# dernasherbrezon/sdr-server

Hardware: AMD Instinct MI355X
Metric: input IQ Msamples/s processed (all clients), 2.016 Msps->48 kHz xlating FIR (higher is better)
Workload: dtype f32; 1 GPU; 1024 clients x 48 kHz off one 2.016 Msps cu8 stream, D=42, 505 taps, 262144-byte blocks (BASELINE configs[3]; N=1: the >=1000-client single-GPU target); clients_total=1024, clients_per_gpu=1024, blocks_per_call=8, mode=optimized, parallelism=single GPU, rccl_ranks=1, feed=xlating_multi (C host)

## Files before the change

### sdr-server_amd/csrc/xl_dev_inline.h

```cpp
#ifndef XL_DEV_INLINE_H_
#define XL_DEV_INLINE_H_
#include "xl_device.h"
#include "xl_q15_narrow.h"

typedef float v2f __attribute__((ext_vector_type(2)));
typedef float v4f __attribute__((ext_vector_type(4)));
typedef const float __attribute__((address_space(4))) *cfloat_p;
typedef const uint32_t __attribute__((address_space(4))) *cu32_p;

#define XL_DEV static __device__ __forceinline__
#define XL_MEM __device__ __forceinline__

XL_DEV v2f xl_sample(const void *__restrict__ p, int fmt, uint32_t i) {
  v2f r;
  if (fmt == XLF_CU8) {
    const uint32_t v = reinterpret_cast<const uint16_t *>(p)[i];
    r.x = ((float)(v & 0xFFu) - 127.5f) / 128.0f;
    r.y = ((float)(v >> 8) - 127.5f) / 128.0f;
  } else if (fmt == XLF_CS8) {
    const int32_t v = reinterpret_cast<const int16_t *>(p)[i];
    r.x = (float)((int32_t)(int8_t)(v & 0xFF)) / 128.0f;
    r.y = (float)(v >> 8) / 128.0f;
  } else if (fmt == XLF_CS16) {
    const int32_t v = reinterpret_cast<const int32_t *>(p)[i];
    r.x = (float)((int32_t)(int16_t)(v & 0xFFFF)) / 32768.0f;
    r.y = (float)(v >> 16) / 32768.0f;
  } else {
    r = reinterpret_cast<const v2f *>(p)[i];
  }
  return r;
}

XL_DEV v2f xl_sample_q15(const void *__restrict__ p, int fmt, uint32_t i) {
  v2f r;
  if (fmt == XLF_CU8) {
    const uint32_t v = reinterpret_cast<const uint16_t *>(p)[i];
    r.x = (float)(((int32_t)(v & 0xFFu) - 128) * 256);
    r.y = (float)(((int32_t)(v >> 8) - 128) * 256);
  } else if (fmt == XLF_CS8) {
    const int32_t v = reinterpret_cast<const int16_t *>(p)[i];
    r.x = (float)((int32_t)(int8_t)(v & 0xFF) * 256);
    r.y = (float)((v >> 8) * 256);
  } else {
    const int32_t v = reinterpret_cast<const int32_t *>(p)[i];
    r.x = (float)(int32_t)(int16_t)(v & 0xFFFF);
    r.y = (float)(v >> 16);
  }
  return r;
}

XL_DEV void xl_q15_rotate_store(const short2 *__restrict__ qphtab, float2 *out, uint32_t off, uint32_t qi, uint32_t m, int32_t ar,
                                int32_t ai) {
  const short2 p0 = qphtab[(off >> XL_PH_SHIFT) + (m >> XL_PH_SHIFT)];
  const int32_t ir = (int16_t)(qi & 0xFFFFu), ii = (int16_t)(qi >> 16);
  int32_t pr = p0.x, pi = p0.y;
  for (uint32_t j = m & (XL_PH_STRIDE - 1u); j > 0u; --j) {
    const int32_t tr = pr * ir - pi * ii, ti = pr * ii + pi * ir;
    pr = xl_sat16(tr >> 15);
    pi = xl_sat16(ti >> 15);
  }
  const int32_t orr = ar * pr - ai * pi, oi = ar * pi + ai * pr;
  reinterpret_cast<short2 *>(out + off)[m] = make_short2((short)xl_sat16(orr >> 15), (short)xl_sat16(oi >> 15));
}

template <int MODE>
struct XlAcc;

template <>
struct XlAcc<0> {
  v2f s;
  XL_MEM void clear() { s = (v2f){0.0f, 0.0f}; }
  XL_MEM void mac(const v2f x, const float hr, const float hi) {
    const v2f h = {hr, hi};
    v2f p1, p2;
    asm("v_pk_mul_f32 %0, %3, %4 op_sel_hi:[0,1]\n\t"
        "v_pk_mul_f32 %1, %3, %4 op_sel:[1,1] op_sel_hi:[1,0]\n\t"
        "v_pk_add_f32 %0, %0, %1 neg_lo:[0,1]\n\t"
        "v_pk_add_f32 %2, %2, %0"
        : "=&v"(p1), "=&v"(p2), "+v"(s)
        : "v"(x), "s"(h));
  }
  XL_MEM v2f value() const { return s; }
};

template <>
struct XlAcc<1> {
  v2f a, b;
  XL_MEM void clear() {
    a = (v2f){0.0f, 0.0f};
    b = (v2f){0.0f, 0.0f};
  }
  XL_MEM void mac(const v2f x, const float hr, const float hi) {
    a = __builtin_elementwise_fma((v2f){x.x, x.x}, (v2f){hr, hi}, a);
    b = __builtin_elementwise_fma((v2f){x.y, x.y}, (v2f){hi, hr}, b);
  }
  XL_MEM v2f value() const { return (v2f){a.x - b.x, a.y + b.y}; }
};

template <int MODE>
XL_DEV v2f xl_rotate(const v2f a, const v2f p) {
  v2f r;
  if (MODE == 0) {
    r.x = a.x * p.x - a.y * p.y;
    r.y = a.x * p.y + a.y * p.x;
  } else {
    r.x = __builtin_fmaf(-a.y, p.y, a.x * p.x);
    r.y = __builtin_fmaf(a.y, p.x, a.x * p.y);
  }
  return r;
}

XL_DEV void xl_nco_step(v2f &p, const v2f inc) {
  v2f t1, t2;
  asm volatile(
      "v_pk_mul_f32 %0, %2, %3 op_sel_hi:[1,0]\n\t"
      "v_pk_mul_f32 %1, %2, %3 op_sel:[0,1] op_sel_hi:[1,1]"
      : "=&v"(t1), "=&v"(t2)
      : "v"(p), "v"(inc));
  asm volatile("v_pk_add_f32 %0, %1, %2 op_sel:[0,1] op_sel_hi:[1,0] neg_lo:[0,1]" : "=v"(p) : "v"(t1), "v"(t2));
}

XL_DEV v2f xl_nco_next(const v2f p, const v2f inc) {
  v2f t1, t2, r;
  asm volatile(
      "v_pk_mul_f32 %0, %3, %4 op_sel_hi:[1,0]\n\t"
      "v_pk_mul_f32 %1, %3, %4 op_sel:[0,1] op_sel_hi:[1,1]\n\t"
      "v_pk_add_f32 %2, %0, %1 op_sel:[0,1] op_sel_hi:[1,0] neg_lo:[0,1]"
      : "=&v"(t1), "=&v"(t2), "=&v"(r)
      : "v"(p), "v"(inc));
  return r;
}

XL_DEV v2f xl_nco_next_fma(const v2f p, const v2f inc) {
  v2f t, r;
  asm volatile(
      "v_pk_mul_f32 %0, %2, %3 op_sel:[1,1] op_sel_hi:[1,0]\n\t"
      "v_pk_fma_f32 %1, %2, %3, %0 op_sel_hi:[0,1,1] neg_lo:[0,0,1]"
      : "=&v"(t), "=&v"(r)
      : "v"(p), "v"(inc));
  return r;
}
XL_DEV v2f xl_nco_next_any(const v2f p, const v2f inc, const uint32_t flags) {
  return (flags & XL_POS_FMA_STEP) ? xl_nco_next_fma(p, inc) : xl_nco_next(p, inc);
}

XL_DEV v2f xl_nco_role_step(const v2f p, const v2f inc, const uint32_t flags) {
  float a, b, c, d;
  if (flags & XL_POS_FMA_STEP) {
    asm volatile(
        "v_mul_f32 %0, %3, %5\n\t"
        "v_mul_f32 %1, %3, %4\n\t"
        "v_fma_f32 %0, %2, %4, -%0\n\t"
        "v_fma_f32 %1, %2, %5, %1"
        : "=&v"(a), "=&v"(b)
        : "v"(p.x), "v"(p.y), "v"(inc.x), "v"(inc.y));
    return (v2f){a, b};
  }
  asm volatile(
      "v_mul_f32 %0, %4, %6\n\t"
      "v_mul_f32 %1, %5, %7\n\t"
      "v_mul_f32 %2, %4, %7\n\t"
      "v_mul_f32 %3, %5, %6\n\t"
      "v_sub_f32 %0, %0, %1\n\t"
      "v_add_f32 %1, %3, %2"
// ... 87 lines not shown
```

### sdr-server_amd/csrc/xl_kernels.hip

```cpp
#include "xl_dev_inline.h"
#include "xl_chain_plan.h"

#include <hip/hip_ext.h>

#include <stdlib.h>

__global__ __launch_bounds__(64) void xl_nco_table_kernel(const XlNcoClient *__restrict__ cl, uint32_t n,
                                                          const float2 *state_in, float2 *state_out,
                                                          float2 *__restrict__ tab, const XlPos pos,
                                                          const uint32_t explicit_K, const uint32_t prio,
                                                          const uint32_t lanes) {
  if (prio == 3) __builtin_amdgcn_s_setprio(3);
  else if (prio == 2) __builtin_amdgcn_s_setprio(2);
  else if (prio == 1) __builtin_amdgcn_s_setprio(1);
  if (threadIdx.x >= lanes) return;
  const uint32_t c = blockIdx.x * lanes + threadIdx.x;
  if (c >= n) return;
  const XlNcoClient k = cl[c];
  const XlBnd bnd = xl_nco_bnd(k, pos, explicit_K);
  asm volatile("" ::: "v255", "a255");
  xl_nco_client_chain<true>(k, bnd, 0u, bnd.K, state_in, state_out, tab);
}

#define XLC_RING 64u
XL_DEV uint32_t xl_lds_off(const void *p) { return (uint32_t)(uintptr_t)(__attribute__((address_space(3))) const char *)p; }
XL_DEV void xl_lds_post(const uint32_t addr, const uint32_t v) { asm volatile("ds_write_b32 %0, %1" ::"v"(addr), "v"(v) : "memory"); }
XL_DEV void xl_lds_post64(const uint32_t addr, const v2f v) { asm volatile("ds_write_b64 %0, %1" ::"v"(addr), "v"(v) : "memory"); }
XL_DEV uint32_t xl_lds_poll(const uint32_t addr) {
  uint32_t v;
  asm volatile("ds_read_b32 %0, %1\n\ts_waitcnt lgkmcnt(0)" : "=v"(v) : "v"(addr) : "memory");
  return v;
}

XL_DEV uint32_t xl_lds_poll3_min(const uint32_t a0, const uint32_t a1, const uint32_t a2) {
  uint32_t v0, v1, v2;
  asm volatile("ds_read_b32 %0, %3\n\tds_read_b32 %1, %4\n\tds_read_b32 %2, %5\n\ts_waitcnt lgkmcnt(0)"
               : "=&v"(v0), "=&v"(v1), "=&v"(v2)
               : "v"(a0), "v"(a1), "v"(a2)
               : "memory");
  v0 = v0 < v1 ? v0 : v1;
  return v0 < v2 ? v0 : v2;
}
XL_DEV uint32_t xl_chain_lim(const uint32_t mn) { return mn >= 0x7FFFFFE0u ? 0xFFFFFFFFu : 2u * mn + XLC_RING; }
XL_DEV uint32_t xl_chain_wait_drained(const uint32_t upto, const uint32_t a0, const uint32_t a1, const uint32_t a2) {
  uint32_t lim = 0u;
  for (uint32_t spin = 0; spin < (1u << 22); ++spin) {
    lim = xl_chain_lim((uint32_t)__builtin_amdgcn_readfirstlane((int)xl_lds_poll3_min(a0, a1, a2)));
    if (upto <= lim) break;
    __builtin_amdgcn_s_sleep(1);
  }
  return lim;
}
XL_DEV uint32_t xl_chain_event(uint32_t ev) {
  const unsigned long long act = __ballot(ev != 0xFFFFFFFFu);
  if (act == 0ull) return 0xFFFFFFFFu;
  const uint32_t first = (uint32_t)__builtin_amdgcn_readlane((int)ev, (int)__ffsll((long long)act) - 1);
  if (__ballot(ev != 0xFFFFFFFFu && ev != first) == 0ull) return first;
#pragma unroll
  for (int sh = 1; sh < 64; sh <<= 1) {
    const uint32_t other = (uint32_t)__shfl_xor((int)ev, sh);
    ev = other < ev ? other : ev;
  }
  return (uint32_t)__builtin_amdgcn_readfirstlane((int)ev);
}

#define XLC_ALIGN ".p2align 6\n\t"
#define XLC_MUL "v_pk_mul_f32 %[t1], %[p], %[inc] op_sel_hi:[1,0]\n\tv_pk_mul_f32 %[t2], %[p], %[inc] op_sel:[0,1] op_sel_hi:[1,1]\n\t"
#define XLC_ADD "v_pk_add_f32 %[p], %[t1], %[t2] op_sel:[0,1] op_sel_hi:[1,0] neg_lo:[0,1]\n\t"
#define XLC_STEP XLC_MUL XLC_ADD
#define XLC_STEP2(I1, I2) XLC_MUL I1 "\n\t" XLC_ADD I2 "\n\t"
#define XLC_STEPS10 XLC_STEP XLC_STEP XLC_STEP XLC_STEP XLC_STEP XLC_STEP XLC_STEP XLC_STEP XLC_STEP XLC_STEP
#define XLC_ANY_LOOP                                                                       \
  "1:\n\t" XLC_MUL "ds_write_b64 %[addr], %[p]\n\t" XLC_ADD                               \
  XLC_STEP2("v_add_u32 %[cnt], 1, %[cnt]", "s_sub_u32 %[todo], %[todo], 1")               \
  XLC_MUL "ds_write_b32 %[paddr], %[cnt]\n\t" XLC_ADD                                     \
  XLC_MUL "v_add_u32 %[off], 0x200, %[off]\n\t" XLC_ADD                                   \
  XLC_MUL "v_and_b32 %[off], 0x7fff, %[off]\n\t" XLC_ADD                                  \
  XLC_STEP2("v_add_u32 %[addr], %[off], %[base]", "s_cmp_lg_u32 %[todo], 0")              \
  XLC_STEPS10 "s_cbranch_scc1 1b\n\t"
#define XLC_B8_LOOP                                                                        \
  "2:\n\t" XLC_E7("0", "512", "1024", "1536", "2048", "2560", "3072")                    \
  XLC_MUL "ds_write_b64 %[addr], %[p] offset:3584\n\t" XLC_ADD                           \
  XLC_STEP2("v_add_u32 %[cnt], 8, %[cnt]", "s_sub_u32 %[todo8], %[todo8], 1")            \
  XLC_MUL "ds_write_b32 %[paddr], %[cnt]\n\t" XLC_ADD                                    \
  XLC_MUL "v_add_u32 %[off], 0x1000, %[off]\n\t" XLC_ADD                                 \
  XLC_MUL "v_and_b32 %[off], 0x7fff, %[off]\n\t" XLC_ADD                                 \
  XLC_STEP2("v_add_u32 %[addr], %[off], %[base]", "s_cmp_lg_u32 %[todo8], 0")            \
  XLC_STEPS10 "s_cbranch_scc1 2b\n\t"
#define XLC_ANY_PART "s_cmp_eq_u32 %[todo], 0\n\ts_cbranch_scc1 3f\n\t" XLC_ANY_LOOP "3:\n\ts_nop 0\n\t"
#define XLC_B8_PART "s_cmp_eq_u32 %[todo8], 0\n\ts_cbranch_scc1 4f\n\t" XLC_B8_LOOP "4:\n\ts_nop 0\n\t"
#define XLC_STEP_LOOP "1:\n\t" XLC_STEP2("s_sub_u32 %[todo], %[todo], 1", "s_cmp_lg_u32 %[todo], 0") "s_cbranch_scc1 1b\n\t"
#define XLC_QENTRY(OFFS) XLC_MUL "ds_write_b64 %[addr], %[p] offset:" OFFS "\n\t" XLC_ADD XLC_STEP XLC_STEP
#define XLC_E(OFFS) XLC_QENTRY(OFFS) XLC_STEP XLC_STEP XLC_STEP XLC_STEPS10
#define XLC_E7(B0, B1, B2, B3, B4, B5, B6) XLC_E(B0) XLC_E(B1) XLC_E(B2) XLC_E(B3) XLC_E(B4) XLC_E(B5) XLC_E(B6)
#define XLC_E8(B0, B1, B2, B3, B4, B5, B6, B7) XLC_E7(B0, B1, B2, B3, B4, B5, B6) XLC_E(B7)
#define XLC_B32_LOOP                                                                                         \
  XLC_E8("0", "512", "1024", "1536", "2048", "2560", "3072", "3584")                                       \
  XLC_E8("4096", "4608", "5120", "5632", "6144", "6656", "7168", "7680")                                   \
  XLC_E8("8192", "8704", "9216", "9728", "10240", "10752", "11264", "11776")                               \
  XLC_E("12288") XLC_E("12800") XLC_E("13312") XLC_E("13824") XLC_E("14336") XLC_E("14848")               \
  XLC_QENTRY("15360")                                                                                      \
  XLC_MUL "ds_read_b32 %[mn], %[an0]\n\t" XLC_ADD                                                           \
  XLC_MUL "ds_read_b32 %[n1], %[an1]\n\t" XLC_ADD                                                           \
  XLC_MUL "ds_read_b32 %[n2], %[an2]\n\t" XLC_ADD XLC_STEPS10                                               \
  XLC_MUL "ds_write_b64 %[addr], %[p] offset:15872\n\t" XLC_ADD                                             \
  XLC_MUL "v_add_u32 %[cnt], 32, %[cnt]\n\t" XLC_ADD "s_sub_u32 %[todo], %[todo], 1\n\t"                    \
  XLC_MUL "ds_write_b32 %[paddr], %[cnt]\n\t" XLC_ADD                                                       \
  XLC_MUL "v_add_u32 %[off], 0x4000, %[off]\n\t" XLC_ADD                                                    \
  XLC_MUL "v_and_b32 %[off], 0x7fff, %[off]\n\t" XLC_ADD                                                    \
  XLC_STEP2("v_add_u32 %[addr], %[off], %[base]", "s_add_u32 %[need], %[need], 16")                         \
  XLC_STEP2("s_waitcnt lgkmcnt(0)", "v_min_u32 %[mn], %[mn], %[n1]")                                        \
  XLC_STEP2("v_min_u32 %[mn], %[mn], %[n2]", "s_nop 0")                                                     \
  XLC_STEP2("v_readfirstlane_b32 %[sm], %[mn]", "s_nop 0")                                                  \
  XLC_STEP2("s_cmp_ge_u32 %[sm], %[need]", "s_cselect_b32 %[st], %[todo], 0")                               \
  XLC_STEP XLC_STEP XLC_STEP XLC_STEP XLC_STEP XLC_STEP
static_assert(XL_PH_STRIDE == 16u && XLC_RING * 64u * 8u == 0x8000u, "the chain wave's asm blocks are written for 16 steps per entry and a 32 KB ring");

__global__ __launch_bounds__(256) void xl_nco_chain_kernel(const XlNcoClient *__restrict__ cl, uint32_t n,
                                                           const float2 *state_in, const XlChainCalls calls,
                                                           XlPos pos, unsigned long long *stats) {
  asm volatile("" ::: "v255", "a255");
  const unsigned long long t_entry = stats ? wall_clock64() : 0ull;
  __shared__ v2f ring[XLC_RING][64];
  __shared__ uint32_t s_emax;
  __shared__ uint32_t s_prod;
  __shared__ uint32_t s_next[3];
  const uint32_t w = __builtin_amdgcn_readfirstlane(threadIdx.x >> 6), lane = threadIdx.x & 63u;
  const uint32_t c = blockIdx.x * 64u + lane;
  const bool have = c < n;
  XlNcoClient k;
  k.incr = make_float2(1.0f, 0.0f);
  k.out_off = 0u, k.slot = 0u, k.D = 1u, k.rem0 = 0u;
  if (have) k = cl[c];
  v2f p = {1.0f, 0.0f};
  if (w == 0 && have) p = (v2f){state_in[k.slot].x, state_in[k.slot].y};
  unsigned long long cyc = 0ull, ticks = 0ull, wfirst = 0ull;
  uint32_t entries = 0u;
  for (uint32_t call = 0; call < calls.n; ++call, pos = xl_grid_next(pos)) {
    float2 *const tab = calls.tab[call];
    float2 *const state_out = calls.state_out[call];
    if (call) __syncthreads();
    XlBnd bnd = xl_nco_bnd(k, pos, 0xFFFFFFFFu);
    if (!have) bnd.K = 0u;
    const uint32_t K = bnd.K, E = (K + XL_PH_STRIDE - 1u) >> XL_PH_SHIFT;
    if (threadIdx.x == 0) {
      s_emax = 0u;
      s_prod = 0u;
      s_next[0] = 0u, s_next[1] = 1u, s_next[2] = 2u;
    }
    __syncthreads();
    if (w == 0 && E > 0u) atomicMax(&s_emax, E);
    __syncthreads();
    const uint32_t Emax = (uint32_t)__builtin_amdgcn_readfirstlane((int)s_emax);
    const uint32_t a_prod = xl_lds_off(&s_prod), a_ring0 = xl_lds_off(&ring[0][0]), a_ring = xl_lds_off(&ring[0][lane]);
    v2f *__restrict__ o = reinterpret_cast<v2f *>(tab) + (k.out_off >> XL_PH_SHIFT);
    if (w == 0) {
      __builtin_amdgcn_s_setprio(3);
      const v2f inc = {k.incr.x, k.incr.y};
      uint32_t nb = xl_bnd_next(bnd, 0u);
      const uint32_t a_n0 = xl_lds_off(&s_next[0]), a_n1 = xl_lds_off(&s_next[1]), a_n2 = xl_lds_off(&s_next[2]);
      const unsigned long long c0 = stats ? clock64() : 0ull, w0 = stats ? wall_clock64() : 0ull;
      unsigned long long t_region = 0ull, t_drain = 0ull, t_b32 = 0ull;
      uint32_t n_drain = 0u, n_b32 = 0u, n_event = 0u, n_runs = 0u;
      uint32_t e = 0;
      uint32_t lim = XLC_RING;
      uint32_t evs = xl_chain_event(0u < K ? (nb < K ? nb : K) : 0xFFFFFFFFu);
      while (e < Emax) {
        uint32_t e_stop = evs == 0u ? 0u : (evs - 1u) >> XL_PH_SHIFT;
        e_stop = e_stop < Emax ? e_stop : Emax;
        if (pos.pad & XL_POS_FMA_STEP) e_stop = e;
        const unsigned long long r0 = stats ? clock64() : 0ull;
        if ((e << XL_PH_SHIFT) < K) {
          const XlChainPlan8 pl = xl_chain_plan8(e, e_stop, XLC_RING, 32u, 8u);
          uint32_t ee = e;
          v2f t1, t2;
#define XLC_COVER_RUN(N1, N8, PARTS)                                                                                         \
  if ((N1) + (N8) != 0u) {                                                                                                   \
    uint32_t todo = (N1), todo8 = (N8);                                                                                      \
    const uint32_t total = todo + 8u * todo8;                                                                                \
    if (ee + total > lim) {                                                                                                  \
      const unsigned long long d0 = stats ? clock64() : 0ull;                                                                \
      lim = xl_chain_wait_drained(ee + total, a_n0, a_n1, a_n2);                                                             \
      if (stats) t_drain += clock64() - d0, ++n_drain;                                                                       \
    }                                                                                                                        \
    uint32_t off = ((ee & (XLC_RING - 1u)) << 9) + lane * (uint32_t)sizeof(v2f);     \
    uint32_t addr = a_ring0 + off, cnt = ee;                                                                                 \
    ee += total;                                                                                                             \
    asm volatile(XLC_ALIGN PARTS                                                                                             \
                 : [p] "+v"(p), [off] "+v"(off), [addr] "+v"(addr), [cnt] "+v"(cnt), [t1] "=&v"(t1), [t2] "=&v"(t2),         \
                   [todo] "+s"(todo), [todo8] "+s"(todo8)                                                                    \
                 : [inc] "v"(inc), [base] "v"(a_ring0), [paddr] "v"(a_prod)                                                  \
                 : "memory", "scc");                                                                                         \
  }
          XLC_COVER_RUN(pl.head1, pl.head8, XLC_ANY_PART XLC_B8_PART);
          for (uint32_t want = pl.blocks; want != 0u;) {
            if (ee + 32u > lim) {
              const unsigned long long d0 = stats ? clock64() : 0ull;
              lim = xl_chain_wait_drained(ee + 32u, a_n0, a_n1, a_n2);
              if (stats) t_drain += clock64() - d0, ++n_drain;
            }
            uint32_t off = ((ee & (XLC_RING - 1u)) << 9) + lane * (uint32_t)sizeof(v2f);
            uint32_t addr = a_ring0 + off, cnt = ee;
            uint32_t left = want, need = (ee >> 1) - 16u, mn, n1, n2, sm, st;
            const unsigned long long b0 = stats ? clock64() : 0ull;
            asm volatile(XLC_ALIGN "1:\n\t" XLC_B32_LOOP "s_cmp_lg_u32 %[st], 0\n\ts_cbranch_scc1 1b\n\t"
                         : [p] "+v"(p), [off] "+v"(off), [addr] "+v"(addr), [cnt] "+v"(cnt), [t1] "=&v"(t1), [t2] "=&v"(t2),
                           [mn] "=&v"(mn), [n1] "=&v"(n1), [n2] "=&v"(n2), [todo] "+s"(left), [need] "+s"(need), [sm] "=&s"(sm),
                           [st] "=&s"(st)
                         : [inc] "v"(inc), [base] "v"(a_ring0), [paddr] "v"(a_prod), [an0] "v"(a_n0), [an1] "v"(a_n1), [an2] "v"(a_n2)
                         : "memory", "scc");
            const uint32_t ran = (want - left) << 5;
            if (stats) t_b32 += clock64() - b0, n_b32 += ran, ++n_runs;
            lim = xl_chain_lim(sm);
            ee += ran;
            want = left;
          }
          XLC_COVER_RUN(pl.tail1, pl.tail8, XLC_B8_PART XLC_ANY_PART);
#undef XLC_COVER_RUN
        }
        if (e_stop > e) e = e_stop;
        if (stats) t_region += clock64() - r0, ++n_event;
        if (e < Emax) {
          if (e + 1u > lim) lim = xl_chain_wait_drained(e + 1u, a_n0, a_n1, a_n2);
          const uint32_t m0 = e << XL_PH_SHIFT;
          if (m0 < K) xl_lds_post64(a_ring + (e & (XLC_RING - 1u)) * 64u * (uint32_t)sizeof(v2f), p);
          xl_lds_post(a_prod, e + 1u);
          uint32_t m = m0;
          if (!(pos.pad & XL_POS_FMA_STEP) && evs - m0 - 1u < XL_PH_STRIDE &&
              __ballot(m0 < K && (nb != evs || m0 + XL_PH_STRIDE > K)) == 0ull && m0 < K) {
            v2f t1, t2;
            uint32_t todo = evs - m0;
            asm volatile(XLC_ALIGN XLC_STEP_LOOP
                         : [p] "+v"(p), [t1] "=&v"(t1), [t2] "=&v"(t2), [todo] "+s"(todo)
                         : [inc] "v"(inc)
                         : "scc");
            p = xl_nco_renorm(p);
            nb = xl_bnd_next(bnd, evs);
            m = evs;
            todo = m0 + XL_PH_STRIDE - evs;
            if (todo != 0u && __ballot(nb <= m0 + XL_PH_STRIDE) == 0ull) {
              asm volatile(XLC_ALIGN XLC_STEP_LOOP
                           : [p] "+v"(p), [t1] "=&v"(t1), [t2] "=&v"(t2), [todo] "+s"(todo)
                           : [inc] "v"(inc)
                           : "scc");
              m = m0 + XL_PH_STRIDE;
            }
          }
          for (; m < m0 + XL_PH_STRIDE && m < K; ++m) {
            p = xl_nco_next_any(p, inc, bnd.flags);
            if (m + 1u == nb) {
              p = xl_nco_renorm(p);
              nb = xl_bnd_next(bnd, m + 1u);
            }
          }
          ++e;
          evs = xl_chain_event((e << XL_PH_SHIFT) < K ? (nb < K ? nb : K) : 0xFFFFFFFFu);
        }
      }
      if (have) state_out[k.slot] = make_float2(p.x, p.y);
      if (stats) {
        cyc += clock64() - c0;
        const unsigned long long w1 = wall_clock64();
        ticks += w1 - w0;
        entries += Emax;
        if (call == 0u) wfirst = w0;
        if (lane == 0u && blockIdx.x < 1024u) {
          stats[8192u + 8u * blockIdx.x + 1u + 2u * call] = w0 - t_entry;
          stats[8192u + 8u * blockIdx.x + 2u + 2u * call] = w1 - t_entry;
        }
        if (lane == 0u && blockIdx.x < 128u) {
          unsigned long long *const sp = stats + 4096u + 32u * blockIdx.x + 8u * call;
          const unsigned long long k0 = clock64(), k1 = clock64(), k2 = clock64(), k3 = clock64(), k4 = clock64();
          (void)k1, (void)k2, (void)k3;
          sp[0] = k0 - c0, sp[1] = t_region, sp[2] = t_drain, sp[3] = t_b32;
          sp[4] = n_drain, sp[5] = n_b32, sp[6] = n_event | ((unsigned long long)n_runs << 32), sp[7] = (k4 - k0) / 4ull;
        }
      }
      continue;
    }
    const uint32_t j = w - 1u;
    const uint32_t a_next = xl_lds_off(&s_next[j]);
    v4f *__restrict__ o4 = reinterpret_cast<v4f *>(o);
    for (uint32_t q = j; 2u * q < Emax; q += 3u) {
      const uint32_t need = 2u * q + 2u < Emax ? 2u * q + 2u : Emax;
      for (uint32_t spin = 0; spin < (1u << 24); ++spin) {
        if (xl_lds_poll(a_prod) >= need) break;
        __builtin_amdgcn_s_sleep(1);
      }
      if (2u * q < E) {
        v2f a, b2 = {0.0f, 0.0f};
        const uint32_t ra = a_ring + ((2u * q) & (XLC_RING - 1u)) * 64u * (uint32_t)sizeof(v2f);
        const uint32_t rb = a_ring + ((2u * q + 1u) & (XLC_RING - 1u)) * 64u * (uint32_t)sizeof(v2f);
        const bool two = 2u * q + 1u < E;
        asm volatile("ds_read_b64 %0, %1" : "=v"(a) : "v"(ra) : "memory");
        if (two) asm volatile("ds_read_b64 %0, %1" : "=v"(b2) : "v"(rb) : "memory");
        asm volatile("s_waitcnt lgkmcnt(0)" ::: "memory");
        if (two) o4[q] = (v4f){a.x, a.y, b2.x, b2.y};
        else o[2u * q] = a;
      }
      xl_lds_post(a_next, q + 3u);
    }
    xl_lds_post(a_next, 0xFFFFFFFFu);
  }
  if (stats) __syncthreads();
  if (stats && threadIdx.x == 0u) {
    if (blockIdx.x < 1024u) {
      stats[8192u + 8u * blockIdx.x] = t_entry;
      stats[8192u + 8u * blockIdx.x + 7u] = wall_clock64() - t_entry;
    }
    stats[4u * blockIdx.x] = cyc;
    stats[4u * blockIdx.x + 1u] = ticks;
    stats[4u * blockIdx.x + 2u] = entries;
    stats[4u * blockIdx.x + 3u] = wfirst;
  }
}

template <int FMT>
XL_DEV void xl_stage_window(const XlFirArgs &a, const uint32_t zero_below, const uint32_t win0, const uint32_t wlen,
                            v2f *__restrict__ win) {
  const uint32_t bd = blockDim.x;
  for (uint32_t j0 = threadIdx.x; j0 < wlen; j0 += 4u * bd) {
    v2f v[4];
    bool ok[4];
#pragma unroll
    for (int u = 0; u < 4; ++u) {
      const uint32_t j = j0 + u * bd;
      const uint32_t s = win0 + j;
      const bool first = s < a.n0;
      ok[u] = j < wlen && s >= zero_below && (first || s - a.n0 < a.n1);
      const void *src = (first || !ok[u]) ? a.in0 : a.in1;
      const uint32_t idx = ok[u] ? (first ? s : s - a.n0) : 0u;
      v[u] = xl_sample(src, FMT, idx);
    }
#pragma unroll
    for (int u = 0; u < 4; ++u) {
      const uint32_t j = j0 + u * bd;
      if (j < wlen) win[j] = ok[u] ? v[u] : (v2f){0.0f, 0.0f};
    }
  }
}

template <int CT, int MODE, bool WIDE>
__global__ __launch_bounds__(64 * XL_NW_MAX) __attribute__((amdgpu_num_sgpr(96))) void xl_fir_kernel(const XlFirArgs a) {
  extern __shared__ __attribute__((aligned(16))) v2f xl_win[];
  const uint32_t OT = a.ota;

  if (blockIdx.x < a.nco_blocks) {
    if (((a.flags >> 4) & 3u) == 3u) __builtin_amdgcn_s_setprio(3);
    else if (((a.flags >> 4) & 3u) == 2u) __builtin_amdgcn_s_setprio(2);
    else if (((a.flags >> 4) & 3u) == 1u) __builtin_amdgcn_s_setprio(1);
    const uint32_t nwave = threadIdx.x >> 6, nlane = threadIdx.x & 63u;
    if (nwave < a.nco_wpw && nlane < XL_NCO_LANES) {
      const unsigned long long t0 = a.trace ? wall_clock64() : 0ull;
      const uint32_t c = (blockIdx.x * a.nco_wpw + nwave) * XL_NCO_LANES + nlane;
      if (c < a.nco_nclients) {
        const XlNcoClient k = a.nco_clients[c];
        const XlBnd bnd = xl_nco_bnd(k, xl_grid_next(a.pos), 0xFFFFFFFFu);
        xl_nco_client_chain<false>(k, bnd, 0u, bnd.K, a.nco_state_in, a.nco_state_out, a.nco_tab);
      }
      if (a.trace && nlane == 0) {
        unsigned long long *tn = a.trace + ((size_t)blockIdx.x * XL_NW_MAX + nwave) * 6;
        tn[0] = t0;
        tn[3] = wall_clock64();
        tn[4] = __builtin_amdgcn_s_getreg((4 << 0) | (0 << 6) | (31 << 11));
        tn[5] = __builtin_amdgcn_s_getreg((20 << 0) | (0 << 6) | (31 << 11));
      }
    }
    return;
  }

  if (!(a.flags & 2u)) __builtin_amdgcn_s_setprio(3);
  const uint32_t b = blockIdx.x - a.nco_blocks;
  const unsigned long long t_entry = a.trace ? wall_clock64() : 0ull;

  const uint32_t roll_blocks = gridDim.x - a.nco_blocks < XL_ROLL_BLOCKS ? gridDim.x - a.nco_blocks : XL_ROLL_BLOCKS;
  if (a.hist_out != nullptr && b < roll_blocks) {
    const uint16_t *__restrict__ h0 = reinterpret_cast<const uint16_t *>(a.in0);
    const uint16_t *__restrict__ h1 = reinterpret_cast<const uint16_t *>(a.in1);
    uint16_t *__restrict__ ho = reinterpret_cast<uint16_t *>(a.hist_out);
    const uint32_t hu = a.hist_units, nu = a.block_units;
    for (uint32_t j = b * blockDim.x + threadIdx.x; j < hu; j += roll_blocks * blockDim.x) {
      const uint32_t sidx = nu + j;
      ho[j] = (sidx < hu) ? h0[sidx] : h1[sidx - hu];
    }
  }
  const uint32_t xcd = b & 7u, idx = b >> 3;
  const uint32_t total = a.ngroups * a.xtiles;
  const uint32_t per = total >> 3, extra = total & 7u;
  const uint32_t len = per + (xcd < extra ? 1u : 0u);
  if (idx >= len) return;
  const uint32_t wi = xcd * per + (xcd < extra ? xcd : extra) + idx;
  const uint32_t y = wi / a.xtiles;
  const uint32_t x = wi - y * a.xtiles;
  if (y >= a.ngroups) return;

  const cu32_p g = (cu32_p)(uintptr_t)(a.groups + y);
  const uint32_t D = g[0], Tpad = g[2], ntiles = g[4];
  const XlDyn d = a.explicit_dyn ? a.dyn1 : xl_grid_dyn(D, g[1], g[3], g[7], a.pos);
  const uint32_t K = d.K;
  const bool live = x * OT < K;
  if (!live && a.nco_lanes == 0u) return;

  const uint32_t w = __builtin_amdgcn_readfirstlane(threadIdx.x >> 6);
  v2f phs[CT];
#pragma unroll
  for (int c = 0; c < CT; ++c) phs[c] = (v2f){1.0f, 0.0f};
  if (live) {
    if (w < ntiles) {
      constexpr uint32_t G = 64u / XL_PH_STRIDE;
      const uint32_t lane = threadIdx.x & 63u;
      v2f *__restrict__ pl = xl_win + w * (CT * 64u);
      const uint32_t *__restrict__ tg = reinterpret_cast<const uint32_t *>(a.groups + y) + 8u + w * XL_TILE_DWORDS;
      const uint32_t c = lane / G, e = lane % G;
      const uint32_t m0 = x * OT + e * XL_PH_STRIDE;
      if (c < tg[1] && e * XL_PH_STRIDE < OT && m0 < K) {
        const uint32_t off = tg[2 + c];
        const float2 ci = reinterpret_cast<const float2 *>(tg + 2 + XL_CT_MAX)[c];
        const uint32_t left = K - m0, span = OT < XL_PH_STRIDE ? OT : XL_PH_STRIDE;
        XlBnd bnd;
        bnd.j0 = d.j0, bnd.D = D, bnd.S = a.pos.S, bnd.G = a.explicit_dyn ? 1u : a.pos.G, bnd.K = K, bnd.flags = a.pos.pad;
        v2f *__restrict__ dst = pl + c * 64u + e * XL_PH_STRIDE;
        xl_phase_walk((reinterpret_cast<const v2f *>(a.phtab) + (off >> XL_PH_SHIFT))[m0 >> XL_PH_SHIFT], m0,
                      left < span ? left : span, (v2f){ci.x, ci.y}, bnd, [&](uint32_t i, v2f ph) { dst[i] = ph; });
      }
      __builtin_amdgcn_wave_barrier();
#pragma unroll
      for (int cc = 0; cc < CT; ++cc) phs[cc] = pl[cc * 64u + lane];
    }
    __syncthreads();

    const uint32_t win0 = d.base + x * OT * D;
    const uint32_t wlen = (OT - 1u) * D + Tpad;
    if (a.fmt == XLF_CU8) xl_stage_window<XLF_CU8>(a, d.zero_below, win0, wlen, xl_win);
    else if (a.fmt == XLF_CS8) xl_stage_window<XLF_CS8>(a, d.zero_below, win0, wlen, xl_win);
// ... 488 lines not shown
```

### sdr-server_amd/csrc/xl_poly_dev.h

```cpp
#ifndef XL_POLY_DEV_H_
#define XL_POLY_DEV_H_
#include "xl_polyphase.h"

#include "xl_dev_inline.h"
#include "xl_fft16.h"

XL_DEV v2f xlp_cmul(const v2f a, const v2f b) {
  return (v2f){__builtin_fmaf(-a.y, b.y, a.x * b.x), __builtin_fmaf(a.y, b.x, a.x * b.y)};
}

struct XlpTw {
  v2f w[3][3];
};
#define XLP_POS(i) ((i) + ((i) >> 2))
#define XLP_ROW(M) ((M) + (M) / 4)
struct XlpPosPad {
  static XL_MEM uint32_t pos(const uint32_t i, const uint32_t) { return XLP_POS(i); }
};
#define XLP_SWZ_ROW(row) ((((row) >> 1) & 15u) ^ (((row) & 1u) << 3))
struct XlpPosSwz {
  static XL_MEM uint32_t pos(const uint32_t i, const uint32_t rs) { return i ^ ((5u * ((i >> 4) & 7u)) & 15u) ^ rs; }
};

template <int SIGN, int M>
XL_DEV XlpTw xlp_twiddles(const v2f *__restrict__ W, const uint32_t l) {
  XlpTw t;
  constexpr int NP4 = M == 256 ? 4 : 3;
#pragma unroll
  for (int pass = 1; pass < NP4; ++pass) {
    const uint32_t p = 1u << (2 * pass);
    const uint32_t k = l & (p - 1u);
    const uint32_t step = 64u >> (2 * pass);
#pragma unroll
    for (int r = 1; r < 4; ++r) {
      v2f w = W[(r * k * step) & 255u];
      if (SIGN > 0) w.y = -w.y;
      t.w[pass - 1][r - 1] = w;
    }
  }
  if (M == 128) {
#pragma unroll
    for (int i = 0; i < 2; ++i) {
      v2f w = W[(2u * l + 64u * i) & 255u];
      if (SIGN > 0) w.y = -w.y;
      t.w[2][i] = w;
    }
  }
  return t;
}

template <int SIGN>
XL_DEV void xlp_dft_butterfly(v2f (&u)[4], const XlpTw &tw, const int pass) {
  if (pass > 0) {
#pragma unroll
    for (int r = 1; r < 4; ++r) u[r] = xlp_cmul(u[r], tw.w[pass - 1][r - 1]);
  }
  const v2f v0 = u[0] + u[2], v1 = u[0] - u[2], v2 = u[1] + u[3], t = u[1] - u[3];
  const v2f v3 = SIGN > 0 ? (v2f){-t.y, t.x} : (v2f){t.y, -t.x};
  u[0] = v0 + v2;
  u[1] = v1 + v3;
  u[2] = v0 - v2;
  u[3] = v1 - v3;
}

template <int SIGN, int NI, int M, class P = XlpPosPad>
XL_DEV void xlp_dft(v2f (&u)[NI][4], v2f *const (&lds)[NI], const XlpTw &tw, const uint32_t l, const uint32_t (&rs)[NI]) {
  constexpr uint32_t L = M / 4;
  constexpr int NP4 = M == 256 ? 4 : 3;
#pragma unroll
  for (int pass = 0; pass < NP4; ++pass) {
    const uint32_t p = 1u << (2 * pass);
    const uint32_t k = l & (p - 1u);
#pragma unroll
    for (int n = 0; n < NI; ++n) xlp_dft_butterfly<SIGN>(u[n], tw, pass);
    if (pass < NP4 - 1 || M == 128) {
      const uint32_t jo = ((l - k) << 2) + k;
#pragma unroll
      for (int n = 0; n < NI; ++n)
#pragma unroll
        for (int r = 0; r < 4; ++r) lds[n][P::pos(jo + r * p, rs[n])] = u[n][r];
      __builtin_amdgcn_wave_barrier();
#pragma unroll
      for (int n = 0; n < NI; ++n)
#pragma unroll
        for (int r = 0; r < 4; ++r) u[n][r] = lds[n][P::pos(l + L * r, rs[n])];
      __builtin_amdgcn_wave_barrier();
    }
  }
  if (M == 128) {
#pragma unroll
    for (int n = 0; n < NI; ++n) {
      const v2f a0 = u[n][0], a1 = xlp_cmul(u[n][2], tw.w[2][0]);
      const v2f b0 = u[n][1], b1 = xlp_cmul(u[n][3], tw.w[2][1]);
      u[n][0] = a0 + a1;
      u[n][1] = b0 + b1;
      u[n][2] = a0 - a1;
      u[n][3] = b0 - b1;
    }
  }
}

typedef _Float16 v8h __attribute__((ext_vector_type(8)));
typedef _Float16 v2h __attribute__((ext_vector_type(2)));
typedef float v16f32 __attribute__((ext_vector_type(16)));

XL_DEV void xlp_lds_barrier() { asm volatile("s_waitcnt lgkmcnt(0)\n\ts_barrier" ::: "memory"); }

XL_DEV uint32_t xlp_seg_exp(const uint32_t maxbits) {
  const uint32_t ex = maxbits >> 23;
  return ex < 27u ? 27u : (ex > 254u ? 254u : ex);
}
XL_DEV float xlp_seg_scale(const uint32_t maxbits) { return __uint_as_float((268u - xlp_seg_exp(maxbits)) << 23); }
XL_DEV float xlp_seg_unscale(const uint32_t maxbits) { return __uint_as_float((xlp_seg_exp(maxbits) - 14u) << 23); }


XL_DEV void xlp_split_h(const float v, _Float16 &h1, _Float16 &h2) {
  h1 = (_Float16)v;
  h2 = (_Float16)(v - (float)h1);
}
XL_DEV uint32_t xlp_pack_h(const _Float16 lo, const _Float16 hi) {
  const v2h p = {lo, hi};
  return __builtin_bit_cast(uint32_t, p);
}

XL_DEV v2f xlp_cmul_s(const v2f v, const v2f cs) {
  v2f r;
  asm("v_pk_mul_f32 %0, %1, %2 op_sel_hi:[1,0]\n\t"
      "v_pk_fma_f32 %0, %1, %2, %0 op_sel:[1,1,0] op_sel_hi:[0,1,1] neg_lo:[1,0,0]"
      : "=&v"(r)
      : "v"(v), "s"(cs));
  return r;
}
XL_DEV v2f xlp_cmul_v(const v2f v, const v2f cs) {
  v2f r;
  asm("v_pk_mul_f32 %0, %1, %2 op_sel_hi:[1,0]\n\t"
      "v_pk_fma_f32 %0, %1, %2, %0 op_sel:[1,1,0] op_sel_hi:[0,1,1] neg_lo:[1,0,0]"
      : "=&v"(r)
      : "v"(v), "v"(cs));
  return r;
}
struct XlpFftOps {
  template <int N>
  static XL_MEM v2f twiddle(const v2f v) {
    return xlp_cmul_s(v, (v2f){xl_w128_cos(N), xl_w128_sin(N)});
  }
  static XL_MEM v2f add_j(const v2f a, const v2f d) {
    v2f r;
    asm("v_pk_add_f32 %0, %1, %2 op_sel:[0,1] op_sel_hi:[1,0] neg_lo:[0,1]" : "=v"(r) : "v"(a), "v"(d));
    return r;
  }
  static XL_MEM v2f sub_j(const v2f a, const v2f d) {
    v2f r;
    asm("v_pk_add_f32 %0, %1, %2 op_sel:[0,1] op_sel_hi:[1,0] neg_hi:[0,1]" : "=v"(r) : "v"(a), "v"(d));
    return r;
  }
};

XL_DEV void xlp_branch_spectrum(const float2 *__restrict__ rt, const uint32_t nlist, const uint32_t j, const uint32_t dl,
                                const uint32_t T, const uint32_t D, const uint32_t A, const uint32_t M, const uint32_t m,
                                const uint32_t b, const double *wc, const double *ws, double &sr, double &si) {
  sr = 0.0, si = 0.0;
  if (b >= D) return;
  for (uint32_t aa = 0; aa < A; ++aa) {
    if (D * aa + b < dl) continue;
    const uint32_t i = D * aa + b - dl;
    if (i >= T) break;
    const uint32_t n = (aa * m) & (M - 1u);
    const double cs = wc[n], sn = ws[n];
    const float2 tv = rt[(size_t)i * nlist + j];
    const double tr = tv.x, ti = tv.y;
    sr += tr * cs - ti * sn;
    si += tr * sn + ti * cs;
  }
}

XL_DEV void xlp_mix_place(const uint32_t bid, const uint32_t M, const uint32_t runs, uint32_t &m, uint32_t &cg, uint32_t &run) {
  const uint32_t grp = bid / (8u * runs), rr = bid - grp * 8u * runs;
  run = rr >> 3;
  const uint32_t per = M >> 3;
  m = (rr & 7u) * per + grp % per, cg = grp / per;
}

XL_DEV void xlp_nco_role(const XlpArgs &a) {
  if (a.nco_prio == 3u) __builtin_amdgcn_s_setprio(3);
  else if (a.nco_prio == 2u) __builtin_amdgcn_s_setprio(2);
  else if (a.nco_prio == 1u) __builtin_amdgcn_s_setprio(1);
  if (threadIdx.x >= XL_NCO_LANES) return;
  const unsigned long long t0 = a.trace ? wall_clock64() : 0ull;
  const uint32_t c = blockIdx.x * XL_NCO_LANES + threadIdx.x;
  if (c >= a.nco_nclients) return;
  const XlNcoClient k = a.nco_clients[c];
  const XlBnd bnd = xl_nco_bnd(k, xl_grid_next(a.pos), 0xFFFFFFFFu);
  const uint32_t K = bnd.K;
  const uint32_t kb = a.nco_k0 == 0u ? 0u : (uint32_t)(((uint64_t)K * a.nco_k0) >> 16) & ~(2u * XL_PH_STRIDE - 1u);
  const uint32_t ke = a.nco_k1 >= 65536u ? K : (uint32_t)(((uint64_t)K * a.nco_k1) >> 16) & ~(2u * XL_PH_STRIDE - 1u);
  unsigned long long st[2] = {0ull, 0ull};
  xl_nco_client_chain<false>(k, bnd, kb, ke, a.nco_state_src, a.nco_state_dst, a.nco_tab, a.trace ? st : nullptr);
  if (a.trace && threadIdx.x == 0) {
    unsigned long long *t = a.trace + 8 + 8 * blockIdx.x;
    t[0] = t0;
    t[1] = st[0];
    t[2] = st[1];
    t[3] = wall_clock64();
    t[4] = ke - kb;
    t[5] = ((unsigned long long)__builtin_amdgcn_s_getreg((20 << 0) | (0 << 6) | (31 << 11)) << 32) |
           __builtin_amdgcn_s_getreg((4 << 0) | (0 << 6) | (31 << 11));
  }
}

XL_DEV bool xlp_work_role_or_skip(const XlpArgs &a) {
  if (blockIdx.x < a.nco_blocks) {
    xlp_nco_role(a);
    return true;
  }
  return blockIdx.x >= a.nco_skip_at && blockIdx.x < a.nco_skip_at + a.nco_skip;
}
XL_DEV uint32_t xlp_work_index(const XlpArgs &a) { return blockIdx.x - a.nco_blocks - (blockIdx.x >= a.nco_skip_at ? a.nco_skip : 0u); }
XL_DEV bool xlp_work_block(const XlpArgs &a, uint32_t &bid) {
  if (xlp_work_role_or_skip(a)) return false;
  bid = xlp_work_index(a);
  return true;
}

XL_DEV void xlp_trace_work(const XlpArgs &a, const unsigned long long t0) {
#ifdef XL_TUNING
  if (a.trace && (threadIdx.x & 63u) == 0u) {
    const uint32_t slot = xlp_work_index(a) * (blockDim.x >> 6) + (threadIdx.x >> 6);
    if (slot < 6000u) {
      unsigned long long *t = a.trace + 4096 + 4 * (size_t)slot;
      t[0] = t0;
      t[1] = wall_clock64();
      t[2] = ((unsigned long long)__builtin_amdgcn_s_getreg((20 << 0) | (0 << 6) | (31 << 11)) << 32) |
             __builtin_amdgcn_s_getreg((4 << 0) | (0 << 6) | (31 << 11));
    }
  }
#else
  (void)a;
  (void)t0;
#endif
}

#endif
```

Measured before the change: 5.888 million Msamples/s.

## Precompute per-call NCO bounds and double-buffer chain-kernel LDS sync state

The NCO chain kernel now computes per-call boundary data up front, including the block-wide maximum entry count via wave shuffles. This replaces the per-call LDS atomicMax and the three __syncthreads per call with a single lightweight LDS barrier and double-buffered producer/next counters that consumers re-post for the following call. The step loop is restructured into an odd-step prefix plus a two-step body, and the consumer limit is refreshed from LDS around the renormalisation. This trades extra registers and more complex synchronisation invariants for fewer barriers on the serial NCO critical path.

```diff
diff --git a/sdr-server_amd/csrc/xl_dev_inline.h b/sdr-server_amd/csrc/xl_dev_inline.h
--- a/sdr-server_amd/csrc/xl_dev_inline.h
+++ b/sdr-server_amd/csrc/xl_dev_inline.h
@@ -10,6 +10,8 @@
 
 #define XL_DEV static __device__ __forceinline__
 #define XL_MEM __device__ __forceinline__
+
+XL_DEV void xlp_lds_barrier() { asm volatile("s_waitcnt lgkmcnt(0)\n\ts_barrier" ::: "memory"); }
 
 XL_DEV v2f xl_sample(const void *__restrict__ p, int fmt, uint32_t i) {
   v2f r;
diff --git a/sdr-server_amd/csrc/xl_kernels.hip b/sdr-server_amd/csrc/xl_kernels.hip
--- a/sdr-server_amd/csrc/xl_kernels.hip
+++ b/sdr-server_amd/csrc/xl_kernels.hip
@@ -62,6 +62,20 @@
     ev = other < ev ? other : ev;
   }
   return (uint32_t)__builtin_amdgcn_readfirstlane((int)ev);
+}
+XL_DEV uint32_t xl_chain_emax(uint32_t E) {
+  const uint32_t first = (uint32_t)__builtin_amdgcn_readfirstlane((int)E);
+  if (__ballot(E != first) == 0ull) return first;
+#pragma unroll
+  for (int sh = 1; sh < 64; sh <<= 1) {
+    const uint32_t other = (uint32_t)__shfl_xor((int)E, sh);
+    E = other > E ? other : E;
+  }
+  return (uint32_t)__builtin_amdgcn_readfirstlane((int)E);
+}
+XL_DEV void xl_shift4(uint32_t (&v)[XL_CHAIN_MAXCALLS]) {
+#pragma unroll
+  for (uint32_t i = 0; i + 1u < XL_CHAIN_MAXCALLS; ++i) v[i] = v[i + 1u];
 }
 
 #define XLC_ALIGN ".p2align 6\n\t"
@@ -89,7 +103,11 @@
   XLC_STEPS10 "s_cbranch_scc1 2b\n\t"
 #define XLC_ANY_PART "s_cmp_eq_u32 %[todo], 0\n\ts_cbranch_scc1 3f\n\t" XLC_ANY_LOOP "3:\n\ts_nop 0\n\t"
 #define XLC_B8_PART "s_cmp_eq_u32 %[todo8], 0\n\ts_cbranch_scc1 4f\n\t" XLC_B8_LOOP "4:\n\ts_nop 0\n\t"
-#define XLC_STEP_LOOP "1:\n\t" XLC_STEP2("s_sub_u32 %[todo], %[todo], 1", "s_cmp_lg_u32 %[todo], 0") "s_cbranch_scc1 1b\n\t"
+#define XLC_STEP_LOOP                                                                                                  \
+  "s_cmp_eq_u32 %[todo1], 0\n\ts_cbranch_scc1 1f\n\t" XLC_STEP                                                       \
+  "1:\n\ts_cmp_eq_u32 %[todo2], 0\n\ts_cbranch_scc1 3f\n\t"                                                          \
+  "2:\n\t" XLC_STEP2("s_sub_u32 %[todo2], %[todo2], 1", "s_cmp_lg_u32 %[todo2], 0") XLC_STEP "s_cbranch_scc1 2b\n\t" \
+  "3:\n\ts_nop 0\n\t"
 #define XLC_QENTRY(OFFS) XLC_MUL "ds_write_b64 %[addr], %[p] offset:" OFFS "\n\t" XLC_ADD XLC_STEP XLC_STEP
 #define XLC_E(OFFS) XLC_QENTRY(OFFS) XLC_STEP XLC_STEP XLC_STEP XLC_STEPS10
 #define XLC_E7(B0, B1, B2, B3, B4, B5, B6) XLC_E(B0) XLC_E(B1) XLC_E(B2) XLC_E(B3) XLC_E(B4) XLC_E(B5) XLC_E(B6)
@@ -122,43 +140,57 @@
   asm volatile("" ::: "v255", "a255");
   const unsigned long long t_entry = stats ? wall_clock64() : 0ull;
   __shared__ v2f ring[XLC_RING][64];
-  __shared__ uint32_t s_emax;
-  __shared__ uint32_t s_prod;
-  __shared__ uint32_t s_next[3];
+  __shared__ uint32_t s_prod[2];
+  __shared__ uint32_t s_next[2][3];
   const uint32_t w = __builtin_amdgcn_readfirstlane(threadIdx.x >> 6), lane = threadIdx.x & 63u;
   const uint32_t c = blockIdx.x * 64u + lane;
   const bool have = c < n;
   XlNcoClient k;
   k.incr = make_float2(1.0f, 0.0f);
   k.out_off = 0u, k.slot = 0u, k.D = 1u, k.rem0 = 0u;
-  if (have) k = cl[c];
   v2f p = {1.0f, 0.0f};
-  if (w == 0 && have) p = (v2f){state_in[k.slot].x, state_in[k.slot].y};
+  if (have) {
+    k = cl[c];
+    p = (v2f){state_in[k.slot].x, state_in[k.slot].y};
+  }
+  uint32_t c_j0[XL_CHAIN_MAXCALLS], c_K[XL_CHAIN_MAXCALLS], c_nb[XL_CHAIN_MAXCALLS], c_emax[XL_CHAIN_MAXCALLS];
+  {
+    XlPos pc = pos;
+#pragma unroll
+    for (uint32_t i = 0; i < XL_CHAIN_MAXCALLS; ++i, pc = xl_grid_next(pc)) {
+      c_j0[i] = c_K[i] = c_nb[i] = c_emax[i] = 0u;
+      if (i < calls.n) {
+        XlBnd b = xl_nco_bnd(k, pc, 0xFFFFFFFFu);
+        if (!have) b.K = 0u;
+        c_j0[i] = b.j0, c_K[i] = b.K;
+        c_nb[i] = xl_bnd_next(b, 0u);
+        c_emax[i] = xl_chain_emax((b.K + XL_PH_STRIDE - 1u) >> XL_PH_SHIFT);
+      }
+    }
+  }
+  const uint32_t a_ring0 = xl_lds_off(&ring[0][0]), a_ring = xl_lds_off(&ring[0][lane]);
+  if (w != 0) {
+    xl_lds_post(xl_lds_off(&s_next[0][w - 1u]), w - 1u);
+    if (w == 1) xl_lds_post(xl_lds_off(&s_prod[0]), 0u);
+  }
   unsigned long long cyc = 0ull, ticks = 0ull, wfirst = 0ull;
   uint32_t entries = 0u;
-  for (uint32_t call = 0; call < calls.n; ++call, pos = xl_grid_next(pos)) {
+  for (uint32_t call = 0; call < calls.n; ++call, xl_shift4(c_j0), xl_shift4(c_K), xl_shift4(c_nb), xl_shift4(c_emax)) {
     float2 *const tab = calls.tab[call];
     float2 *const state_out = calls.state_out[call];
-    if (call) __syncthreads();
-    XlBnd bnd = xl_nco_bnd(k, pos, 0xFFFFFFFFu);
-    if (!have) bnd.K = 0u;
+    xlp_lds_barrier();
+    const uint32_t par = call & 1u;
+    XlBnd bnd;
+    bnd.j0 = c_j0[0], bnd.D = k.D, bnd.S = pos.S, bnd.G = pos.G, bnd.K = c_K[0], bnd.flags = pos.pad;
     const uint32_t K = bnd.K, E = (K + XL_PH_STRIDE - 1u) >> XL_PH_SHIFT;
-    if (threadIdx.x == 0) {
-      s_emax = 0u;
-      s_prod = 0u;
-      s_next[0] = 0u, s_next[1] = 1u, s_next[2] = 2u;
-    }
-    __syncthreads();
-    if (w == 0 && E > 0u) atomicMax(&s_emax, E);
-    __syncthreads();
-    const uint32_t Emax = (uint32_t)__builtin_amdgcn_readfirstlane((int)s_emax);
-    const uint32_t a_prod = xl_lds_off(&s_prod), a_ring0 = xl_lds_off(&ring[0][0]), a_ring = xl_lds_off(&ring[0][lane]);
+    const uint32_t Emax = (uint32_t)__builtin_amdgcn_readfirstlane((int)c_emax[0]);
+    const uint32_t a_prod = xl_lds_off(&s_prod[par]);
     v2f *__restrict__ o = reinterpret_cast<v2f *>(tab) + (k.out_off >> XL_PH_SHIFT);
     if (w == 0) {
       __builtin_amdgcn_s_setprio(3);
       const v2f inc = {k.incr.x, k.incr.y};
-      uint32_t nb = xl_bnd_next(bnd, 0u);
-      const uint32_t a_n0 = xl_lds_off(&s_next[0]), a_n1 = xl_lds_off(&s_next[1]), a_n2 = xl_lds_off(&s_next[2]);
+      uint32_t nb = c_nb[0];
+      const uint32_t a_n0 = xl_lds_off(&s_next[par][0]), a_n1 = xl_lds_off(&s_next[par][1]), a_n2 = xl_lds_off(&s_next[par][2]);
       const unsigned long long c0 = stats ? clock64() : 0ull, w0 = stats ? wall_clock64() : 0ull;
       unsigned long long t_region = 0ull, t_drain = 0ull, t_b32 = 0ull;
       uint32_t n_drain = 0u, n_b32 = 0u, n_event = 0u, n_runs = 0u;
@@ -229,22 +261,32 @@
           if (!(pos.pad & XL_POS_FMA_STEP) && evs - m0 - 1u < XL_PH_STRIDE &&
               __ballot(m0 < K && (nb != evs || m0 + XL_PH_STRIDE > K)) == 0ull && m0 < K) {
             v2f t1, t2;
-            uint32_t todo = evs - m0;
-            asm volatile(XLC_ALIGN XLC_STEP_LOOP
-                         : [p] "+v"(p), [t1] "=&v"(t1), [t2] "=&v"(t2), [todo] "+s"(todo)
-                         : [inc] "v"(inc)
-                         : "scc");
+#define XLC_RUN_STEPS(N)                                                                                           \
+  {                                                                                                                \
+    uint32_t todo1 = (N) & 1u, todo2 = (N) >> 1;                                                                   \
+    asm volatile(XLC_ALIGN XLC_STEP_LOOP                                                                           \
+                 : [p] "+v"(p), [t1] "=&v"(t1), [t2] "=&v"(t2), [todo2] "+s"(todo2)                                \
+                 : [inc] "v"(inc), [todo1] "s"(todo1)                                                              \
+                 : "scc");                                                                                         \
+  }
+            XLC_RUN_STEPS(evs - m0);
+            uint32_t d0, d1, d2;
+            asm volatile("ds_read_b32 %0, %3\n\tds_read_b32 %1, %4\n\tds_read_b32 %2, %5"
+                         : "=&v"(d0), "=&v"(d1), "=&v"(d2)
+                         : "v"(a_n0), "v"(a_n1), "v"(a_n2)
+                         : "memory");
             p = xl_nco_renorm(p);
             nb = xl_bnd_next(bnd, evs);
+            asm volatile("s_waitcnt lgkmcnt(0)" : "+v"(d0), "+v"(d1), "+v"(d2)::"memory");
+            d0 = d0 < d1 ? d0 : d1;
+            lim = xl_chain_lim((uint32_t)__builtin_amdgcn_readfirstlane((int)(d0 < d2 ? d0 : d2)));
             m = evs;
-            todo = m0 + XL_PH_STRIDE - evs;
-            if (todo != 0u && __ballot(nb <= m0 + XL_PH_STRIDE) == 0ull) {
-              asm volatile(XLC_ALIGN XLC_STEP_LOOP
-                           : [p] "+v"(p), [t1] "=&v"(t1), [t2] "=&v"(t2), [todo] "+s"(todo)
-                           : [inc] "v"(inc)
-                           : "scc");
+            const uint32_t rest = m0 + XL_PH_STRIDE - evs;
+            if (rest != 0u && __ballot(nb <= m0 + XL_PH_STRIDE) == 0ull) {
+              XLC_RUN_STEPS(rest);
               m = m0 + XL_PH_STRIDE;
             }
+#undef XLC_RUN_STEPS
           }
           for (; m < m0 + XL_PH_STRIDE && m < K; ++m) {
             p = xl_nco_next_any(p, inc, bnd.flags);
@@ -279,7 +321,9 @@
       continue;
     }
     const uint32_t j = w - 1u;
-    const uint32_t a_next = xl_lds_off(&s_next[j]);
+    const uint32_t a_next = xl_lds_off(&s_next[par][j]);
+    xl_lds_post(xl_lds_off(&s_next[par ^ 1u][j]), j);
+    if (j == 0u) xl_lds_post(xl_lds_off(&s_prod[par ^ 1u]), 0u);
     v4f *__restrict__ o4 = reinterpret_cast<v4f *>(o);
     for (uint32_t q = j; 2u * q < Emax; q += 3u) {
       const uint32_t need = 2u * q + 2u < Emax ? 2u * q + 2u : Emax;
diff --git a/sdr-server_amd/csrc/xl_poly_dev.h b/sdr-server_amd/csrc/xl_poly_dev.h
--- a/sdr-server_amd/csrc/xl_poly_dev.h
+++ b/sdr-server_amd/csrc/xl_poly_dev.h
@@ -104,7 +104,6 @@
 typedef _Float16 v2h __attribute__((ext_vector_type(2)));
 typedef float v16f32 __attribute__((ext_vector_type(16)));
 
-XL_DEV void xlp_lds_barrier() { asm volatile("s_waitcnt lgkmcnt(0)\n\ts_barrier" ::: "memory"); }
 
 XL_DEV uint32_t xlp_seg_exp(const uint32_t maxbits) {
   const uint32_t ex = maxbits >> 23;
```

Measured after the change: 5.889 million Msamples/s (median of 3 runs). No clear change (+0.0%).
